# facebookresearch/SlowFast

Measured on AMD Instinct MI355X. Metric: clips/sec (fwd+bwd), SlowFast-8x8-R50 32x224^2 synthetic clips, per-GPU batch 32, higher is better.
Workload: dtype fp16; 1 GPU; SLOWFAST_8x8_R50: forward + cross_entropy loss + backward + sgd step, inputs resident in HBM, per-GPU batch 32; global_batch=32, parallelism=dp1, launch=hip-graph(fwd+bwd) + eager all-reduce/optimizer, optimizer=FlatOptimizer (fused unscale+norm+clip+update, dynamic loss scale on device)

## Files before the change

include/sfamd.h:

```cpp
#ifndef SFAMD_H
#define SFAMD_H
#include <stddef.h>
#include <stdint.h>
#ifdef __cplusplus
extern "C" {
#endif

#define SF_ABI_VERSION 32
typedef void* sf_stream_t;

typedef struct sf_conv_desc {
    int32_t N, Ci, Ti, Hi, Wi;
    int32_t Co, To, Ho, Wo;
    int32_t kT, kH, kW;
    int32_t sT, sH, sW;
    int32_t pT, pH, pW;
    int32_t dT, dH, dW;
    int32_t Cw;
    int32_t ldx, ldy;
    int32_t Cow;
} sf_conv_desc;

int sf_abi_version(void);
const char* sf_backend(void);
#define SF_ACT_FP16 0
#define SF_ACT_BF16_ID 1
int sf_act_dtype(void);
const char* sf_last_error(void);
const char* sf_build_id(void);

int sf_conv_weight_ld(const sf_conv_desc* d, int32_t* ldf, int32_t* ldd);
int sf_prep_weights(const sf_conv_desc* d, const float* w, void* wf, void* wd, sf_stream_t stream);
typedef struct sf_prep_item {
    const float* w;
    void* wf;
    void* wd;
    int32_t Co, Cow, Cw, Cp, taps, ldf, ldd;
    int32_t pad;
} sf_prep_item;
int sf_prep_item_fill(const sf_conv_desc* d, const float* w, void* wf, void* wd, sf_prep_item* item);
int64_t sf_prep_item_blocks(const sf_prep_item* item);
// ... 286 lines not shown
```

slowfast_amd/csrc/sf_api.hip:

```cpp
#include "../../include/sfamd.h"
#include "sf_bn.h"
#include "sf_common.h"
#include "sf_igemm.h"
#include "sf_igemm2.h"
#include "sf_wgrad2.h"
#include "sf_cbwd.h"
#include "sf_pool.h"
#include "sf_dwconv.h"
#include "sf_dwsweep.h"
#include "sf_dwtemporal.h"
#include "sf_tokens.h"
#include "sf_x3d.h"
#include "sf_stem.h"
#include "sf_attn.h"
#include "sf_roi.h"
#include "sf_optim.h"
#include "sf_mixup.h"
#include "sf_erase.h"
#include "sf_pack.h"
#include "sf_sample.h"
#include "sf_color.h"
#include "sf_randaug.h"
#include "sf_hog.h"
#include "sf_pixel.h"
// ... 837 lines not shown
    r.lanes = lanes;
    const int per_block = SF_THREADS / lanes;
    hipLaunchKernelGGL(sf_wgrad_reduce_kernel, dim3(cdiv(total, per_block)), dim3(SF_THREADS), 0, s, r);
    return check_launch("wgrad_reduce");
}

struct CbwdPlan {
    bool ok;
    int cip, cop, R;
    size_t ws_bytes;
};
#define SF_CBWD_MAX_WGS 1024
template <int CIP, int COP>
static void cbwd_fill(CbwdPlan& w) {
    using K = CbwdCfg<CIP, COP>;
    w.R = K::R;
    w.ws_bytes = (size_t)SF_CBWD_MAX_WGS * COP * CIP * 4;
}
#define SF_CBWD_FOR_SHAPE(cip, cop, ...)                                                         \
    do {                                                                                         \
        if ((cip) == 16 && (cop) == 32) { constexpr int CIP_ = 16, COP_ = 32; __VA_ARGS__; }            \
        else if ((cip) == 16 && (cop) == 64) { constexpr int CIP_ = 16, COP_ = 64; __VA_ARGS__; }       \
        else if ((cip) == 16 && (cop) == 128) { constexpr int CIP_ = 16, COP_ = 128; __VA_ARGS__; }     \
        else if ((cip) == 16 && (cop) == 256) { constexpr int CIP_ = 16, COP_ = 256; __VA_ARGS__; }     \
        else if ((cip) == 32 && (cop) == 32) { constexpr int CIP_ = 32, COP_ = 32; __VA_ARGS__; }       \
        else if ((cip) == 32 && (cop) == 64) { constexpr int CIP_ = 32, COP_ = 64; __VA_ARGS__; }       \
        else if ((cip) == 32 && (cop) == 128) { constexpr int CIP_ = 32, COP_ = 128; __VA_ARGS__; }     \
        else if ((cip) == 32 && (cop) == 256) { constexpr int CIP_ = 32, COP_ = 256; __VA_ARGS__; }     \
        else if ((cip) == 64 && (cop) == 32) { constexpr int CIP_ = 64, COP_ = 32; __VA_ARGS__; }       \
        else if ((cip) == 64 && (cop) == 64) { constexpr int CIP_ = 64, COP_ = 64; __VA_ARGS__; }       \
        else if ((cip) == 64 && (cop) == 128) { constexpr int CIP_ = 64, COP_ = 128; __VA_ARGS__; }     \
        else { constexpr int CIP_ = 64, COP_ = 256; __VA_ARGS__; }                                      \
    } while (0)
static CbwdPlan plan_cbwd(const sf_conv_desc* d, bool in_affine, bool mask_bits) {
    CbwdPlan w;
    memset(&w, 0, sizeof(w));
    if (test_hook("SF_CBWD", 1) == 0) return w;
    if (d->kT != 1 || d->kH != 1 || d->kW != 1 || d->sT != 1 || d->sH != 1 || d->sW != 1 || d->pT || d->pH || d->pW) return w;
    if (d->To != d->Ti || d->Ho != d->Hi || d->Wo != d->Wi) return w;
    if (d->Ci % 8 || d->Ci > 64 || d->Co % 32 || d->Co > 256) return w;
    if (in_affine || !mask_bits) return w;
    w.cip = d->Ci <= 16 ? 16 : d->Ci <= 32 ? 32 : 64;
    w.cop = d->Co <= 32 ? 32 : d->Co <= 64 ? 64 : d->Co <= 128 ? 128 : 256;
    SF_CBWD_FOR_SHAPE(w.cip, w.cop, (cbwd_fill<CIP_, COP_>(w)));
    w.ok = true;
    return w;
}

extern "C" int sf_conv_c_bwd_plan(const sf_conv_desc* d, int in_affine, int mask_bits, int32_t* tile_rows,
                                  int64_t* workspace_bytes) {
    if (check_desc(d)) return -1;
    const CbwdPlan w = plan_cbwd(d, in_affine != 0, mask_bits != 0);
    if (tile_rows) *tile_rows = w.ok ? 128 : 0;
    if (workspace_bytes) *workspace_bytes = w.ok ? (int64_t)w.ws_bytes : 0;
    return w.ok ? 1 : 0;
}

extern "C" int sf_conv_c_bwd(const sf_conv_desc* d, const void* dz, int32_t lddz, const void* mask_bits, const void* yc,
                             int32_t ldyc, const float* coef, const void* act, const void* wd, const float* bn_scale,
                             const float* bn_shift, const void* bn_y, int32_t bn_ldy, float* bn_part, int32_t bn_part_rows,
                             int32_t* bn_rows, void* d_in, int32_t ld_in, float* dw, float out_scale, int zero_first,
                             void* workspace, int64_t workspace_bytes, sf_stream_t stream) {
    if (check_desc(d)) return -1;
    REQUIRE(dz && mask_bits && yc && coef && act && wd && d_in && dw && workspace, "sf_conv_c_bwd: null pointer");
    const CbwdPlan w = plan_cbwd(d, false, true);
    REQUIRE(w.ok, "sf_conv_c_bwd: this geometry keeps sf_bn_bwd_apply + sf_conv_wgrad + sf_conv_dgrad_bn (sf_conv_c_bwd_plan == 0)");
    REQUIRE(lddz >= d->Co && lddz % 8 == 0 && ldyc >= d->Co && ldyc % 8 == 0 && ld_in >= d->Ci && ld_in % 8 == 0,
            "sf_conv_c_bwd: bad row pitch");
    REQUIRE((((uintptr_t)dz | (uintptr_t)yc | (uintptr_t)act | (uintptr_t)wd | (uintptr_t)d_in | (uintptr_t)workspace) & 15) == 0,
            "sf_conv_c_bwd: operands must be 16-byte aligned");
    REQUIRE(workspace_bytes >= (int64_t)w.ws_bytes, "sf_conv_c_bwd: workspace too small (%lld < %lld bytes)",
            (long long)workspace_bytes, (long long)w.ws_bytes);
    const int64_t M = (int64_t)d->N * d->Ti * d->Hi * d->Wi;
    const int ntiles = cdiv(M, 128);
    const bool fuse = bn_part != nullptr;
    if (fuse) {
        REQUIRE(bn_scale && bn_shift && bn_y && bn_rows, "sf_conv_c_bwd: the fused reduction needs bn_scale, bn_shift, bn_y and bn_rows");
        REQUIRE(bn_ldy >= d->Ci && bn_ldy % 8 == 0 && ((uintptr_t)bn_y & 15) == 0, "sf_conv_c_bwd: bad bn_y pitch / alignment");
        REQUIRE(bn_part_rows >= ntiles, "sf_conv_c_bwd: the partial table needs ceil(positions / tile_rows) rows of [2][Ci] floats");
    }
    int32_t ldf, ldd;
    sf_conv_weight_ld(d, &ldf, &ldd);
    CbwdParams p;
    memset(&p, 0, sizeof(p));
    p.M = (int)M; p.Ci = d->Ci; p.Co = d->Co;
    p.dz = (const f16*)dz; p.lddz = lddz; p.bits = (const uint8_t*)mask_bits; p.yc = (const f16*)yc; p.ldyc = ldyc;
    p.coef = coef; p.act = (const f16*)act; p.ldact = d->ldx; p.wd = (const f16*)wd; p.ldw = ldd;
    if (fuse) { p.bnb_y = (const f16*)bn_y; p.bnb_ld = bn_ldy; p.bnb_scale = bn_scale; p.bnb_shift = bn_shift; p.bnb_part = bn_part; }
    p.dx = (f16*)d_in; p.lddx = ld_in; p.ws = (float*)workspace; p.tiles128 = ntiles;
    int wgs;
    const Wgrad2Plan w2 = plan_wgrad2(d);
    const int forced = test_hook("SF_CBWD_WGS", 0);
    if (forced > 0) {
        wgs = forced < SF_CBWD_MAX_WGS ? forced : SF_CBWD_MAX_WGS;
        p.rps = roundup(cdiv(M, wgs), 32);
        wgs = cdiv(M, p.rps);
    } else if (w2.ok && w2.thin && w2.splits <= SF_CBWD_MAX_WGS) {
        wgs = w2.splits; p.rps = 0;
    } else {
        const WgradPlan w1 = plan_wgrad(d);
        wgs = w1.splits; p.rps = w1.chunks_per_split * 32;
        REQUIRE(wgs <= SF_CBWD_MAX_WGS, "sf_conv_c_bwd: %d splits", wgs);
    }
    hipStream_t s = (hipStream_t)stream;
    SF_CBWD_FOR_SHAPE(w.cip, w.cop, hipLaunchKernelGGL((sf_cbwd_kernel<CIP_, COP_>), dim3(wgs), dim3(SF_THREADS), 0, s, p));
    if (check_launch("conv_c_bwd")) return -1;
    if (bn_rows) *bn_rows = fuse ? ntiles : 0;
    WgradReduceParams r;
    memset(&r, 0, sizeof(r));
    r.ws = (const float*)workspace; r.splits = wgs; r.Co = d->Cow ? d->Cow : d->Co; r.Co_pad = w.cop; r.Kpad = w.cip;
    r.Ktot = d->Ci; r.fdC = make_fastdiv(d->Ci); r.dw = dw; r.Cw = d->Cw; r.taps = 1; r.slice4 = 0;
    r.out_scale = out_scale; r.accumulate = zero_first ? 0 : 1;
    const int64_t total = (int64_t)r.Co * r.Kpad / 4;
    int lanes = 1;
    while (lanes < 32 && lanes * 4 <= r.splits) lanes *= 2;
    r.lanes = lanes;
    hipLaunchKernelGGL(sf_wgrad_reduce_kernel, dim3(cdiv(total, SF_THREADS / lanes)), dim3(SF_THREADS), 0, s, r);
    return check_launch("conv_c_bwd_reduce");
}

static RowTile make_rowtile(int64_t M, int C, int max_blocks, dim3& grid) {
    RowTile rt;
    rt.M = (int)M; rt.C = C;
    const int G = C / 8;
    const int TG = G < SF_THREADS ? G : SF_THREADS;
    const int rpi = SF_THREADS / TG;
    int passes = cdiv(M, (int64_t)rpi * max_blocks);
    if (passes < 1) passes = 1;
    rt.rows_per_block = rpi * passes;
    grid = dim3(cdiv(M, rt.rows_per_block), cdiv(G, SF_THREADS));
    return rt;
}
static int check_rows(const char* who, int64_t M, int C) {
    REQUIRE(M > 0 && M < (1ll << 31), "%s: bad row count", who);
    REQUIRE(C > 0 && C % 8 == 0, "%s: C must be a positive multiple of 8 (got %d)", who, C);
    return 0;
}

// ... 2264 lines not shown
```

slowfast_amd/csrc/sf_cbwd.h:

```cpp
#pragma once
#include "sf_bn.h"
#include "sf_common.h"
#include "sf_igemm.h"

struct CbwdParams {
    int M, Ci, Co;
    const f16* dz; int lddz;
    const uint8_t* bits;
    const f16* yc; int ldyc;
    const float* coef;
    const f16* act; int ldact;
    const f16* wd; int ldw;
    const f16* bnb_y; int bnb_ld;
    const float* bnb_scale; const float* bnb_shift;
    float* bnb_part;
    f16* dx; int lddx;
    float* ws;
    int rps;
    int tiles128;
};

template <int CIP, int COP>
struct CbwdCfg {
    static constexpr int R = COP >= 128 ? 64 : 128;
    static constexpr int NSUB = 128 / R;
    static constexpr int NJ = CIP / 16, KS = COP / 32, TI = R / 64;
    static constexpr int WAVES_M = COP == 32 ? 4 : 1, WAVES_C = 4 / WAVES_M;
    static constexpr int TC = COP / 16 / WAVES_C;
    static constexpr int KSM = R / WAVES_M / 32;
    static constexpr int LDY = COP + 8;
    static constexpr int CGO = COP / 8, RPP = SF_THREADS / CGO, NCH = R / RPP;
    static constexpr int ACH = CIP / 8, NACT = R * ACH / 64;
    static constexpr int NEPI = (R * ACH + SF_THREADS - 1) / SF_THREADS;
    static constexpr int DY_ELEMS = R * LDY, ACT_ELEMS = R * CIP, WD_ELEMS = CIP * LDY;
    static constexpr int RED_ELEMS = 4 * ACH * 24 * 2;
    static constexpr int UNION_ELEMS = DY_ELEMS > ACT_ELEMS + RED_ELEMS ? DY_ELEMS : ACT_ELEMS + RED_ELEMS;
    static constexpr int LDS_ELEMS = UNION_ELEMS + ACT_ELEMS + WD_ELEMS + 3 * COP * 2 + 2 * CIP * 2;
    static_assert(WAVES_M == 1 || LDS_ELEMS * 2 >= 4 * (COP / 16) * NJ * 256 * 4, "the cross-wave sum reuses the tile buffers");
    static constexpr int LDS_BYTES = LDS_ELEMS * 2;
    static constexpr int HELD = 4 * NJ * (TI + TC) + 9 * NCH + 4 * NEPI;
    static constexpr int OCC = HELD <= 72 ? 3 : 2;
    static_assert(R % 64 == 0 && R % RPP == 0 && NACT >= 1 && (R * ACH) % 64 == 0, "tile shape");
    static_assert(SF_THREADS % ACH == 0 && 64 % ACH == 0, "a thread keeps one d_in column group");
};

template <int CIP, int COP>
__global__ __launch_bounds__(SF_THREADS, (CbwdCfg<CIP, COP>::OCC)) void sf_cbwd_kernel(CbwdParams p) {
    using K = CbwdCfg<CIP, COP>;
    constexpr int R = K::R, LDY = K::LDY, NJ = K::NJ, TI = K::TI, TC = K::TC;
    __shared__ __attribute__((aligned(16))) f16 smem[K::LDS_ELEMS];
    f16* const DyL = smem;
    f16* const StL = smem;
    float* const red = reinterpret_cast<float*>(smem + K::ACT_ELEMS);
    f16* const ActL = smem + K::UNION_ELEMS;
    f16* const WdL = ActL + K::ACT_ELEMS;
    float* const coefL = reinterpret_cast<float*>(WdL + K::WD_ELEMS);
    float* const bnL = coefL + 3 * COP;

    const int tid = threadIdx.x;
    const int lane = tid & 63, wave = __builtin_amdgcn_readfirstlane(tid >> 6);
    const int pl = lane & 15, g4 = lane >> 4;
    const int G = (int)gridDim.x;
    const f16* const zline = reinterpret_cast<const f16*>(sf_zero_line);
    const bool bnb = p.bnb_part != nullptr;

    for (int q = tid; q < CIP * K::CGO; q += SF_THREADS) {
        const int ci = q / K::CGO, cg = q % K::CGO;
        f16x8 v = zero8();
        if (ci < p.Ci && cg * 8 < p.Co) v = ld16(p.wd + (int64_t)ci * p.ldw + cg * 8);
        st16(WdL + ci * LDY + cg * 8, v);
    }
    for (int q = tid; q < 3 * COP; q += SF_THREADS) {
        const int k = q / COP, c = q % COP;
        coefL[q] = c < p.Co ? p.coef[k * p.Co + c] : 0.f;
    }
    for (int q = tid; q < 2 * CIP; q += SF_THREADS) {
        const int k = q / CIP, c = q % CIP;
        bnL[q] = (bnb && c < p.Ci) ? (k ? p.bnb_shift[c] : p.bnb_scale[c]) : (k ? 0.f : 1.f);
    }

    const int scg = tid % K::CGO, srow = tid / K::CGO;
    const bool scol_ok = scg * 8 < p.Co;
    const int scgc = scol_ok ? scg : 0;
    const int ecg = tid % K::ACH;
    const bool ecol_ok = ecg * 8 < p.Ci;
    const int ecgc = ecol_ok ? ecg : 0;

    int r0 = 0, r1 = p.M, T0 = (int)blockIdx.x, Tstep = G, nwalk = 0;
    if (p.rps > 0) {
        r0 = (int)blockIdx.x * p.rps;
        r1 = r0 + p.rps < p.M ? r0 + p.rps : p.M;
        T0 = r0 >> 7;
        Tstep = 1;
        if (r1 > r0) nwalk = (((r1 + 127) >> 7) - T0) * K::NSUB;
    } else if (T0 < p.tiles128) nwalk = ((p.tiles128 - 1 - T0) / G + 1) * K::NSUB;
    auto tile_m0 = [&](int q) { return (T0 + (q / K::NSUB) * Tstep) * 128 + (q % K::NSUB) * R; };

    f16x8 dzr[K::NCH], ycr[K::NCH], ybr[K::NEPI];
    uint32_t mbr[K::NCH];
    auto load_regs = [&](int m0) {
#pragma unroll
        for (int u = 0; u < K::NCH; ++u) {
            int m = m0 + srow + u * K::RPP;
            if (m > p.M - 1) m = p.M - 1;
            dzr[u] = ld16(p.dz + (int64_t)m * p.lddz + scgc * 8);
            ycr[u] = ld16(p.yc + (int64_t)m * p.ldyc + scgc * 8);
            mbr[u] = p.bits[(int64_t)m * (p.Co >> 3) + scgc];
        }
    };
    auto load_yb = [&](int m0) {
#pragma unroll
        for (int e = 0; e < K::NEPI; ++e) {
            int m = m0 + (tid + e * SF_THREADS) / K::ACH;
            if (m > p.M - 1) m = p.M - 1;
            ybr[e] = ld16(p.bnb_y + (int64_t)m * p.bnb_ld + ecgc * 8);
        }
    };
    auto issue_act = [&](int m0) {
#pragma unroll
        for (int j = 0; j < (K::NACT + 3) / 4; ++j) {
            const int q = wave + 4 * j;
            if (q < K::NACT) {
                const int c = q * 64 + lane;
                const int m = m0 + c / K::ACH, cc = c % K::ACH;
                const f16* g = (m >= r0 && m < r1 && cc * 8 < p.Ci) ? p.act + (int64_t)m * p.ldact + cc * 8 : zline;
                SF_GLOBAL_LOAD_LDS16_ASM(g, ActL + q * 512);
            }
        }
    };


    f32x4 wacc[TC][NJ];
#pragma unroll
    for (int i = 0; i < TC; ++i)
#pragma unroll
        for (int j = 0; j < NJ; ++j) wacc[i][j] = (f32x4){0.f, 0.f, 0.f, 0.f};
    const int wc = wave % K::WAVES_C, wm = wave / K::WAVES_C;
    const int cobase = wc * TC * 16, mbase = wm * (R / K::WAVES_M);
    const int rowbase = wave * (R / 4);

    float bsg[8], bsgy[8];
#pragma unroll
    for (int e = 0; e < 8; ++e) { bsg[e] = 0.f; bsgy[e] = 0.f; }
    const int nq = nwalk;
    if (nq > 0) { load_regs(tile_m0(0)); issue_act(tile_m0(0)); }
    for (int q = 0; q < nq; ++q) {
        const int m0 = tile_m0(q);
        const int T = T0 + (q / K::NSUB) * Tstep;
        const bool owner = T * 128 >= r0 && T * 128 < r1;
        const bool more = q + 1 < nq;
        SF_WAIT_VMEM();
        __syncthreads();
        {
            float k1[8], k2[8], k3[8];
#pragma unroll
            for (int e = 0; e < 8; ++e) { k1[e] = coefL[scg * 8 + e]; k2[e] = coefL[COP + scg * 8 + e]; k3[e] = coefL[2 * COP + scg * 8 + e]; }
#pragma unroll
            for (int u = 0; u < K::NCH; ++u) {
                const int row = srow + u * K::RPP;
                const uint32_t b = mbr[u];
                const f16x8 yv = ycr[u];
                float g[8];
#pragma unroll
                for (int e = 0; e < 8; ++e) g[e] = (float)dzr[u][e];
#pragma unroll
                for (int e = 0; e < 8; ++e) g[e] = ((b >> e) & 1u) ? g[e] : 0.f;
                f16x8 o;
#pragma unroll
                for (int e = 0; e < 8; ++e) o[e] = (f16)(k1[e] * g[e] + k2[e] + k3[e] * (float)yv[e]);
                if (!(scol_ok && m0 + row < p.M)) o = zero8();
                st16(DyL + row * LDY + scg * 8, o);
            }
        }
        __syncthreads();
        if (more) load_regs(tile_m0(q + 1));
#pragma unroll
        for (int ks = 0; ks < K::KSM; ++ks) {
            f16x8 af[TC], bf[NJ];
#pragma unroll
            for (int h = 0; h < 2; ++h) {
                const int m = mbase + ks * 32 + 8 * g4 + 4 * h + (pl >> 2);
#pragma unroll
                for (int i = 0; i < TC; ++i) {
                    const f16x4 v = as_f16x4(SF_LDS_TR16(DyL + m * LDY + cobase + i * 16 + 4 * (pl & 3)));
                    af[i][4 * h + 0] = v[0]; af[i][4 * h + 1] = v[1]; af[i][4 * h + 2] = v[2]; af[i][4 * h + 3] = v[3];
                }
#pragma unroll
                for (int j = 0; j < NJ; ++j) {
                    const f16x4 v = as_f16x4(SF_LDS_TR16(ActL + m * CIP + j * 16 + 4 * (pl & 3)));
                    bf[j][4 * h + 0] = v[0]; bf[j][4 * h + 1] = v[1]; bf[j][4 * h + 2] = v[2]; bf[j][4 * h + 3] = v[3];
                }
            }
#pragma unroll
            for (int i = 0; i < TC; ++i)
#pragma unroll
                for (int j = 0; j < NJ; ++j) wacc[i][j] = SF_MFMA16(af[i], bf[j], wacc[i][j]);
        }
        SF_BARRIER_KEEP_VMEM();
        if (more) issue_act(tile_m0(q + 1));
        if (!owner) continue;
        if (bnb) load_yb(m0);
        f32x4 dacc[TI][NJ];
#pragma unroll
        for (int i = 0; i < TI; ++i)
#pragma unroll
            for (int j = 0; j < NJ; ++j) dacc[i][j] = (f32x4){0.f, 0.f, 0.f, 0.f};
#pragma unroll
        for (int ks = 0; ks < K::KS; ++ks) {
            f16x8 bf[NJ];
#pragma unroll
            for (int j = 0; j < NJ; ++j) bf[j] = ld16(WdL + (j * 16 + pl) * LDY + ks * 32 + 8 * g4);
#pragma unroll
            for (int i = 0; i < TI; ++i) {
                const f16x8 af = ld16(DyL + (rowbase + i * 16 + pl) * LDY + ks * 32 + 8 * g4);
#pragma unroll
                for (int j = 0; j < NJ; ++j) dacc[i][j] = SF_MFMA16(af, bf[j], dacc[i][j]);
            }
        }
        SF_BARRIER_KEEP_VMEM();
#pragma unroll
        for (int i = 0; i < TI; ++i)
#pragma unroll
            for (int j = 0; j < NJ; ++j)
#pragma unroll
                for (int r = 0; r < 4; ++r) StL[(rowbase + i * 16 + 4 * g4 + r) * CIP + j * 16 + pl] = (f16)dacc[i][j][r];
        SF_BARRIER_KEEP_VMEM();
        float bsc[8], bsh[8];
#pragma unroll
        for (int e = 0; e < 8; ++e) { bsc[e] = bnL[ecg * 8 + e]; bsh[e] = bnL[CIP + ecg * 8 + e]; }
#pragma unroll
        for (int e = 0; e < K::NEPI; ++e) {
            const int idx = tid + e * SF_THREADS;
            const int row = idx / K::ACH, m = m0 + row;
            if (idx < R * K::ACH && m < p.M && ecol_ok) {
                const f16x8 v = ld16(StL + row * CIP + ecg * 8);
                st16(p.dx + (int64_t)m * p.lddx + ecg * 8, v);
                if (bnb) bnb_accumulate(v, ybr[e], bsc, bsh, bsg, bsgy, false, 0u);
            }
        }
        if (bnb && q % K::NSUB == K::NSUB - 1) {
            bnb_reduce_store<4, K::ACH>(bsg, bsgy, red, p.bnb_part + (int64_t)T * 2 * p.Ci, 0, p.Ci);
#pragma unroll
            for (int e = 0; e < 8; ++e) { bsg[e] = 0.f; bsgy[e] = 0.f; }
        }
    }

    float* slab = p.ws + (int64_t)blockIdx.x * (COP * CIP);
    if constexpr (K::WAVES_M == 4) {
        __syncthreads();
        float* rd = reinterpret_cast<float*>(smem);
#pragma unroll
        for (int i = 0; i < TC; ++i)
#pragma unroll
            for (int j = 0; j < NJ; ++j)
#pragma unroll
                for (int r = 0; r < 4; ++r) rd[(((wave * TC + i) * NJ + j) * 4 + r) * 64 + lane] = wacc[i][j][r];
        __syncthreads();
        constexpr int TE = TC * NJ * 256;
// ... 16 lines not shown
```

slowfast_amd/engine.py:

```python
import functools
import os

import torch

from . import lib as _sflib

from . import ops

_f16 = _sflib.act_dtype()
_listeners = []
FORCE_WEIGHT_PREP = False
PARAM_EPOCH = 0
PACK_RECORD = None
PACK_PLAN = os.environ.get("SF_PACK_PLAN", "1") != "0"
BN_FUSE_REDUCE = os.environ.get("SF_BN_FUSE_REDUCE", "1") != "0"
CAT_IN_PLACE = os.environ.get("SF_CAT_IN_PLACE", "1") != "0"
SEGMENTS = None


class _Segments:
    def __init__(self):
        self.cuts = []

    def cut(self, tensors):
# ... 336 lines not shown
        bn = self.bn
        if bn is None:
            y, _ = ops.conv_fwd(x, wf, geom, in_affine=in_affine, bias=self.conv.bias, stats=False)
            return y, None
        use_batch_stats = training or bn.running_mean is None
        y, part = ops.conv_fwd(x, wf, geom, in_affine=in_affine, bias=self.conv.bias, stats=use_batch_stats)
        return y, bn_statistics(bn, part, geom.out_rows, geom.Co, training)

    def backward(self, x, in_affine, dy, need_dx, resid=None, resid_bits=None, bn_fuse=None):
        geom = self.geom(x.shape)
        w = self.conv.weight
        if w.requires_grad:
            dw, zero_first = _grad_dest(w)
            ops.conv_wgrad(x, dy, geom, dw, in_affine=in_affine, out_scale=1.0, zero_first=zero_first)
        if not need_dx:
            return None
        _, wd = self.weights(geom)
        if bn_fuse is not None:
            if isinstance(bn_fuse, dict):
                return ops.conv_dgrad(dy, wd, geom, resid=resid, resid_bits=resid_bits, bn=bn_fuse)
            y, st = bn_fuse
            return ops.conv_dgrad(dy, wd, geom, resid=resid, bn=(y, st.scale, st.shift))
        return ops.conv_dgrad(dy, wd, geom, resid=resid, resid_bits=resid_bits)

    def _bn_grad_dest(self):
        bn = self.bn
        if bn.weight.requires_grad:
            dgamma, zg = _grad_dest(bn.weight)
            dbeta, zb = _grad_dest(bn.bias)
            assert zg == zb
            return dgamma, dbeta, not zg
        return torch.empty_like(bn.weight), torch.empty_like(bn.bias), False

    def fused_c_geom(self, x):
        if self.bn is None or _sync_of(self.bn) is not None or not self.conv.weight.requires_grad:
            return None
        geom = self.geom(x.shape)
        return geom if ops.conv_c_bwd_plan(geom) is not None else None

    def fused_c_backward(self, geom, x, dz, y, st, bits, part=None, bn_fuse=None):
        bn = self.bn
        dgamma, dbeta, accumulate = self._bn_grad_dest()
        coef = ops.bn_bwd_coef(dz, y, bn.weight, st.mean, st.rstd, dgamma, dbeta, zmask=bits, inv_loss_scale=1.0,
                               accumulate=accumulate, part=part)
        dw, zero_first = _grad_dest(self.conv.weight)
        _, wd = self.weights(geom)
        fuse = None
        if bn_fuse is not None:
            y0, st0 = bn_fuse
            fuse = (y0, st0.scale, st0.shift)
        return ops.conv_c_bwd(dz, bits, y, coef, x, wd, geom, dw, bn=fuse, out_scale=1.0, zero_first=zero_first)

    def bn_backward(self, dz, y, st, zmask=None, relu_self=False, want_g=False, part=None):
        bn = self.bn
        dgamma, dbeta, accumulate = self._bn_grad_dest()
        return ops.bn_bwd(dz, y, bn.weight, st.mean, st.rstd, dgamma, dbeta, zmask=zmask,
                          relu_affine=(st.scale, st.shift) if relu_self else None, inv_loss_scale=1.0,
                          accumulate=accumulate, want_g=want_g, sync=_sync_of(bn), part=part)

    def params(self):
        p = [self.conv.weight]
        if self.conv.bias is not None:
            p.append(self.conv.bias)
        if self.bn is not None:
            p += [self.bn.weight, self.bn.bias]
        return p

    def _fold_source(self, w):
        return w

    def fold(self):
        w = self.conv.weight.detach().float()
        b = self.conv.bias.detach().float() if self.conv.bias is not None else None
        bn = self.bn
        if bn is not None:
            assert bn.running_mean is not None, "BatchNorm without running statistics cannot be folded"
            scale = torch.rsqrt(bn.running_var.detach().float() + bn.eps)
            if bn.weight is not None:
                scale = scale * bn.weight.detach().float()
            shift = -bn.running_mean.detach().float() * scale
            if bn.bias is not None:
                shift = shift + bn.bias.detach().float()
            w = w * scale.view(-1, 1, 1, 1, 1)
            b = shift if b is None else b * scale + shift
# ... 135 lines not shown
            ops.bn_act(x_s, out=cat[:, :Cs])
        ops.bn_act(yf, st.scale, st.shift, relu=True, out=cat[:, Cs:])
        if CAPTURE is not None:
            CAPTURE.append({"kind": "fuse", "mod": mod, "raw": [yf], "bn": [(st.scale, st.shift)]})
        ctx.mod, ctx.yf, ctx.st, ctx.Cs = mod, yf, st, Cs
        ctx.save_for_backward(x_f)
        return cat, x_f.view_as(x_f)

    @staticmethod
    @delivers_grads
    def backward(ctx, dcat, dxf):
        unit = ctx.mod._unit
        (x_f,) = ctx.saved_tensors
        dcat = as_cl(dcat)
        dyf = unit.bn_backward(dcat[:, ctx.Cs:], ctx.yf, ctx.st, relu_self=True)
        need_dx = ctx.needs_input_grad[1]
        dx_f = unit.backward(x_f, None, dyf, need_dx=need_dx, resid=as_cl(dxf) if dxf is not None else None)
        _notify(unit.params())
        ctx.yf = None
        dx_s = dcat[:, :ctx.Cs] if ctx.needs_input_grad[0] else None
        return (dx_s, dx_f, None) + param_grads(ctx, 3)


class ResBlockFn(torch.autograd.Function):

    @staticmethod
    def forward(ctx, x, mod, *params):
        record_params(ctx, params)
        ctx.prev_bn = getattr(x, "_sf_block_bn", None) if BN_FUSE_REDUCE else None
        x = as_cl(x)
        units, P = mod.branch2._chain, mod._proj
        tr = mod.training
        raw, bn, act, h = [], [], [], x
        for i, u in enumerate(units):
            h, st = u.forward(h, None, tr)
            raw.append(h)
            bn.append(st)
            if i + 1 < len(units):
                h = ops.bn_act(h, st.scale, st.shift, relu=True)
                act.append(h)
        yc, sc = raw[-1], bn[-1]
        out_view, cat = None, None
        extra = getattr(mod, "_cat_extra", 0)
        if extra and CAT_IN_PLACE:
            N_, C_, T_, H_, W_ = yc.shape
            cat = ops.cl_empty((N_, C_ + extra, T_, H_, W_), x.device)
            out_view = cat[:, :C_]
        if P is not None:
            y1, s1 = P.forward(x, None, tr)
            out, bits = ops.bn_act(yc, sc.scale, sc.shift, relu=True, resid=y1, rscale=s1.scale, rshift=s1.shift,
                                   want_mask=True, out=out_view)
        else:
            y1, s1 = None, None
            out, bits = ops.bn_act(yc, sc.scale, sc.shift, relu=True, resid=x, want_mask=True, out=out_view)
        if cat is not None:
            out._sf_cat = cat
        if CAPTURE is not None:
            CAPTURE.append({"kind": "resblock", "mod": mod, "raw": list(raw), "bn": [(b.scale, b.shift) for b in bn], "out": out})
        ctx.mod = mod
        ctx.raw = (raw, y1, act, bits)
        ctx.bn = (bn, s1)
        ctx.save_for_backward(x)
        if BN_FUSE_REDUCE and tr:
            out._sf_block_bn = {"bits": bits, "y0": yc, "sync": _sync_of(units[-1].bn) is not None}
        return out

    @staticmethod
    @delivers_grads
    def backward(ctx, dout):
        mod = ctx.mod
        units, P = mod.branch2._chain, mod._proj
        (x,) = ctx.saved_tensors
        raw, y1, act, bits = ctx.raw
        bn, s1 = ctx.bn
        last = len(units) - 1
        part_c = tagged_bn_part(dout, raw[last])
        dout = as_cl(dout)
        need_dx = ctx.needs_input_grad[0]
        cgeom = units[last].fused_c_geom(act[last - 1]) if last > 0 else None
        if cgeom is None:
            dy = units[last].bn_backward(dout, raw[last], bn[last], zmask=bits, part=part_c)
        if P is not None:
            dy1 = P.bn_backward(dout, y1, s1, zmask=bits)
        for i in range(last, 0, -1):
            part = None
            if i == last and cgeom is not None:
                inner = (raw[i - 1], bn[i - 1]) if BN_FUSE_REDUCE and _sync_of(units[i - 1].bn) is None else None
                d_in, part = units[i].fused_c_backward(cgeom, act[i - 1], dout, raw[i], bn[i], bits, part=part_c, bn_fuse=inner)
            elif BN_FUSE_REDUCE and _sync_of(units[i - 1].bn) is None:
                d_in, part = units[i].backward(act[i - 1], None, dy, need_dx=True, bn_fuse=(raw[i - 1], bn[i - 1]))
            else:
                d_in = units[i].backward(act[i - 1], None, dy, need_dx=True)
            dy = units[i - 1].bn_backward(d_in, raw[i - 1], bn[i - 1], relu_self=True, part=part)
        prev = ctx.prev_bn if need_dx else None
        if prev is not None and prev["sync"]:
            prev = None
        if P is not None:
            dx1 = P.backward(x, None, dy1, need_dx=need_dx)
            dx = units[0].backward(x, None, dy, need_dx=need_dx, resid=dx1, bn_fuse=prev)
        else:
            dx = units[0].backward(x, None, dy, need_dx=need_dx, resid=dout, resid_bits=bits, bn_fuse=prev)
        if prev is not None:
            dx, pc = dx
            if pc is not None:
                tag_bn_part(dx, prev["y0"], pc)
        _notify(mod._param_list)
        ctx.raw = ctx.bn = ctx.prev_bn = None
        return (dx, None) + param_grads(ctx, 2)


CUT_BACKWARD = False
_cut_bn_tags = {}


def retag_cut_grad(g):
    tag = _cut_bn_tags.pop(g.data_ptr(), None)
    if tag is not None and getattr(g, "_sf_bn_part", None) is None and tag[2] == g.data_ptr() and tag[3] == g._version:
        g._sf_bn_part = tag


def tag_bn_part(dx, y0, part):
    dx._sf_bn_part = (y0.data_ptr(), part, dx.data_ptr(), dx._version)
    if CUT_BACKWARD:
        _cut_bn_tags[dx.data_ptr()] = dx._sf_bn_part


def tagged_bn_part(dout, y0):
    tag = getattr(dout, "_sf_bn_part", None)
    if tag is None or tag[0] != y0.data_ptr() or tag[2] != dout.data_ptr() or tag[3] != dout._version:
        return None
    return tag[1]


class ConvBNActFn(torch.autograd.Function):

    @staticmethod
    def forward(ctx, x, unit, relu, training, *params):
        record_params(ctx, params)
        x = as_cl(x)
        y, st = unit.forward(x, None, training)
# ... 18 lines not shown
```

slowfast_amd/lib.py:

```python
import ctypes
import os
from ctypes import POINTER, Structure, c_char_p, c_float, c_int, c_int32, c_int64, c_void_p

_HERE = os.path.dirname(os.path.abspath(__file__))
ABI_VERSION = 32
ACT_MODE = os.environ.get("SF_ACT_DTYPE", "fp16").lower()
if ACT_MODE not in ("fp16", "bf16"):
    raise ValueError(f"SF_ACT_DTYPE={ACT_MODE!r}: expected fp16 or bf16")
DEFAULT_LIBRARY = os.path.join(_HERE, "libsfamd.so" if ACT_MODE == "fp16" else "libsfamd_bf16.so")


def act_dtype():
    import torch
    return torch.float16 if ACT_MODE == "fp16" else torch.bfloat16


def act_eps():
    return 2.0 ** -11 if ACT_MODE == "fp16" else 2.0 ** -8


class ConvDesc(Structure):

    _fields_ = [(n, c_int32) for n in (
        "N", "Ci", "Ti", "Hi", "Wi", "Co", "To", "Ho", "Wo", "kT", "kH", "kW", "sT", "sH", "sW",
        "pT", "pH", "pW", "dT", "dH", "dW", "Cw", "ldx", "ldy", "Cow")]


class PrepItem(Structure):

    _fields_ = [("w", c_void_p), ("wf", c_void_p), ("wd", c_void_p)] + [(n, c_int32) for n in (
        "Co", "Cow", "Cw", "Cp", "taps", "ldf", "ldd", "pad")]


class DwDesc(Structure):

    _fields_ = [(n, c_int32) for n in (
        "N", "C", "Cw", "cls", "Ti", "Hi", "Wi", "To", "Ho", "Wo", "kT", "kH", "kW", "sT", "sH", "sW",
        "pT", "pH", "pW", "ldx", "ldy", "Cwreal")]
# ... 237 lines not shown
```

slowfast_amd/ops.py:

```python
from ctypes import byref, c_int32, c_int64

import torch

from . import lib as _sflib

from .lib import ConvDesc, SfError, get_lib

_f16 = _sflib.act_dtype()


def _triple(v):
    return tuple(v) if isinstance(v, (tuple, list)) else (v, v, v)


def _stream(t):
    if t.is_cuda:
        return torch.cuda.current_stream(t.device).cuda_stream
    if get_lib().backend != "hostsim":
        raise SfError("slowfast_amd kernels need CUDA/HIP tensors (got a CPU tensor and the gfx950 library)")
    return None


def _ptr(t):
    return None if t is None else t.data_ptr()
# ... 326 lines not shown
        import torch.distributed as dist
        group, gsize = sync
        tot = part.sum(0, keepdim=True)
        loc = tot.clone()
        lib.call("sf_bn_bwd_finalize", loc.data_ptr(), 1, C, gamma.numel(), float(M), gamma.data_ptr(), mean.data_ptr(),
                 rstd.data_ptr(), float(inv_loss_scale), dgamma.data_ptr(), dbeta.data_ptr(), int(accumulate),
                 coef.data_ptr(), s)
        dist.all_reduce(tot, group=group)
        scratch = torch.empty((2, gamma.numel()), dtype=torch.float32, device=y.device)
        lib.call("sf_bn_bwd_finalize", tot.data_ptr(), 1, C, gamma.numel(), float(M) * gsize, gamma.data_ptr(),
                 mean.data_ptr(), rstd.data_ptr(), float(inv_loss_scale), scratch[0].data_ptr(), scratch[1].data_ptr(), 0,
                 coef.data_ptr(), s)
    if coef_only:
        return coef
    dy = cl_empty(y.shape, y.device) if out is None else out
    if sample_add is not None:
        assert fused_part is not None and zmask is None and relu_affine is None and not want_g
        assert sample_add.dtype == torch.float32 and sample_add.is_contiguous() and tuple(sample_add.shape) == (N, C)
        lib.call("sf_bn_bwd_apply_sample", M, C, dz.data_ptr(), lddz, y.data_ptr(), ldy, coef.data_ptr(), sample_add.data_ptr(),
                 M // N, dy.data_ptr(), cl_ld(dy), s, work=dict(bytes=2.0 * y.numel() * 3))
        return dy
    g = cl_empty(y.shape, y.device) if want_g else None
    lib.call("sf_bn_bwd_apply", M, C, dz.data_ptr(), lddz, _ptr(zmask), ldm, y.data_ptr(), ldy, _ptr(sc), _ptr(sh),
             relu_self, coef.data_ptr(), dy.data_ptr(), cl_ld(dy), _ptr(g), cl_ld(g) if g is not None else 0, s,
             work=dict(bytes=2.0 * y.numel() * (3 + mcost + int(want_g))))
    return (dy, g) if want_g else dy


def bn_bwd_coef(dz, y, gamma, mean, rstd, dgamma, dbeta, zmask=None, inv_loss_scale=1.0, accumulate=False, part=None):
    return bn_bwd(dz, y, gamma, mean, rstd, dgamma, dbeta, zmask=zmask, inv_loss_scale=inv_loss_scale, accumulate=accumulate,
                  part=part, coef_only=True)


def conv_c_bwd_plan(geom, in_affine=False, mask_bits=True):
    tile_rows, ws = c_int32(0), c_int64(0)
    ok = get_lib().call("sf_conv_c_bwd_plan", byref(geom.desc(geom.Ci, geom.Co)), int(bool(in_affine)), int(bool(mask_bits)),
                        byref(tile_rows), byref(ws))
    return (tile_rows.value, ws.value) if ok == 1 else None


def conv_c_bwd(dz, bits, yc, coef, act, wd, geom, dw, bn=None, out_scale=1.0, zero_first=True, out=None):
    plan = conv_c_bwd_plan(geom)
    assert plan is not None, "conv_c_bwd: the planner rejects this geometry"
    tile_rows, ws_bytes = plan
    assert tuple(act.shape) == geom.in_shape and tuple(dz.shape) == geom.out_shape and tuple(yc.shape) == geom.out_shape
    assert dw.dtype == torch.float32 and dw.is_contiguous() and dw.numel() == geom.Cow * geom.Cw * geom.taps
    M = rows(yc)
    assert bits.dtype == torch.uint8 and bits.is_contiguous() and bits.numel() == M * (geom.Co // 8)
    assert coef.dtype == torch.float32 and coef.is_contiguous() and tuple(coef.shape) == (3, geom.Co)
    d_in = cl_empty(geom.in_shape, dz.device) if out is None else out
    assert tuple(d_in.shape) == geom.in_shape
    part, cap, nrows = None, 0, c_int32(0)
    y0 = sc = sh = None
    if bn is not None:
        y0, sc, sh = bn
        assert tuple(y0.shape) == geom.in_shape
        cap = (M + tile_rows - 1) // tile_rows
        part = torch.empty((cap, 2, geom.Ci), dtype=torch.float32, device=dz.device)
    ws = _workspace(dz.device, ws_bytes)
    W = 2.0 * M * geom.Co
    get_lib().call("sf_conv_c_bwd", byref(geom.desc(cl_ld(act), geom.Co)), dz.data_ptr(), cl_ld(dz), bits.data_ptr(), yc.data_ptr(),
                   cl_ld(yc), coef.data_ptr(), act.data_ptr(), wd.data_ptr(), _ptr(sc), _ptr(sh), _ptr(y0),
                   cl_ld(y0) if y0 is not None else 0, _ptr(part), cap, byref(nrows), d_in.data_ptr(), cl_ld(d_in), dw.data_ptr(),
                   float(out_scale), int(zero_first), ws.data_ptr(), ws.numel(), _stream(dz),
                   work=dict(flops=4.0 * M * geom.Co * geom.Cw,
                             bytes=W * (2 + 1 / 16) + 2.0 * M * geom.Ci * (2 + int(bn is not None))))
    return d_in, (part[:nrows.value] if part is not None and nrows.value > 0 else None)


def _pool_args(y, kernel, stride, padding):
    N, C, T, H, W = y.shape
    (kH, kW), (sH, sW), (pH, pW) = kernel, stride, padding
    return (N, T, H, W, C, kH, kW, sH, sW, pH, pW), ((H + 2 * pH - kH) // sH + 1, (W + 2 * pW - kW) // sW + 1)


def pool_fwd(y, kernel, stride, padding, affine=None, want_argmax=True):
    args, (Ho, Wo) = _pool_args(y, kernel, stride, padding)
    N, C, T, H, W = y.shape
    out = cl_empty((N, C, T, Ho, Wo), y.device)
    arg = torch.empty((N, T, Ho, Wo, C), dtype=torch.uint8, device=y.device) if want_argmax else None
    sc, sh, relu = _affine(affine)
    get_lib().call("sf_pool_fwd", *args, y.data_ptr(), cl_ld(y), _ptr(sc), _ptr(sh), relu, out.data_ptr(),
                   cl_ld(out), _ptr(arg), 0, _stream(y), work=dict(bytes=2.0 * (y.numel() + out.numel())))
    return out, arg


def pool_bwd(in_shape, pooled, argmax, dout, kernel, stride, padding, relu=True):
    N, C, T, H, W = in_shape
    (kH, kW), (sH, sW), (pH, pW) = kernel, stride, padding
    assert tuple(dout.shape) == tuple(pooled.shape)
    g = cl_empty(in_shape, dout.device)
    get_lib().call("sf_pool_bwd", N, T, H, W, C, kH, kW, sH, sW, pH, pW, pooled.data_ptr(), cl_ld(pooled),
                   argmax.data_ptr(), int(bool(relu)), dout.data_ptr(), cl_ld(dout), g.data_ptr(), cl_ld(g), 0,
                   _stream(dout), work=dict(bytes=2.0 * (g.numel() + 2.5 * dout.numel())))
    return g
```

Measured before the change: 904.9 clips/s.

## Fold input BN+ReLU into last-unit conv forward and fused backward kernel

In each residual block the last 1x1 conv no longer consumes a materialised BN+ReLU activation. The forward conv takes the affine+relu as an input transform. The fused conv/BN backward kernel gains an AFF variant that recomputes the activation from the raw pre-BN tensor and BN scale/shift into LDS, prefetching the next tile's raw rows. This removes one activation write in forward and one stored tensor, trading it for extra per-element affine work in backward and a different prefetch schedule.

```diff
diff --git a/include/sfamd.h b/include/sfamd.h
--- a/include/sfamd.h
+++ b/include/sfamd.h
@@ -6,7 +6,7 @@
 extern "C" {
 #endif
 
-#define SF_ABI_VERSION 32
+#define SF_ABI_VERSION 33
 typedef void* sf_stream_t;
 
 typedef struct sf_conv_desc {
diff --git a/slowfast_amd/csrc/sf_api.hip b/slowfast_amd/csrc/sf_api.hip
--- a/slowfast_amd/csrc/sf_api.hip
+++ b/slowfast_amd/csrc/sf_api.hip
@@ -893,25 +893,31 @@
         else if ((cip) == 64 && (cop) == 128) { constexpr int CIP_ = 64, COP_ = 128; __VA_ARGS__; }     \
         else { constexpr int CIP_ = 64, COP_ = 256; __VA_ARGS__; }                                      \
     } while (0)
-static CbwdPlan plan_cbwd(const sf_conv_desc* d, bool in_affine, bool mask_bits) {
+static CbwdPlan plan_cbwd_geom(const sf_conv_desc* d) {
     CbwdPlan w;
     memset(&w, 0, sizeof(w));
-    if (test_hook("SF_CBWD", 1) == 0) return w;
     if (d->kT != 1 || d->kH != 1 || d->kW != 1 || d->sT != 1 || d->sH != 1 || d->sW != 1 || d->pT || d->pH || d->pW) return w;
     if (d->To != d->Ti || d->Ho != d->Hi || d->Wo != d->Wi) return w;
     if (d->Ci % 8 || d->Ci > 64 || d->Co % 32 || d->Co > 256) return w;
-    if (in_affine || !mask_bits) return w;
     w.cip = d->Ci <= 16 ? 16 : d->Ci <= 32 ? 32 : 64;
     w.cop = d->Co <= 32 ? 32 : d->Co <= 64 ? 64 : d->Co <= 128 ? 128 : 256;
     SF_CBWD_FOR_SHAPE(w.cip, w.cop, (cbwd_fill<CIP_, COP_>(w)));
     w.ok = true;
     return w;
 }
+static CbwdPlan plan_cbwd(const sf_conv_desc* d, int in_affine, bool mask_bits) {
+    CbwdPlan none;
+    memset(&none, 0, sizeof(none));
+    if (test_hook("SF_CBWD", 1) == 0 || !mask_bits) return none;
+    if (in_affine != 0 && in_affine != 2) return none;
+    if (in_affine == 2 && test_hook("SF_CBWD_AFFINE", 1) == 0) return none;
+    return plan_cbwd_geom(d);
+}
 
 extern "C" int sf_conv_c_bwd_plan(const sf_conv_desc* d, int in_affine, int mask_bits, int32_t* tile_rows,
                                   int64_t* workspace_bytes) {
     if (check_desc(d)) return -1;
-    const CbwdPlan w = plan_cbwd(d, in_affine != 0, mask_bits != 0);
+    const CbwdPlan w = plan_cbwd(d, in_affine, mask_bits != 0);
     if (tile_rows) *tile_rows = w.ok ? 128 : 0;
     if (workspace_bytes) *workspace_bytes = w.ok ? (int64_t)w.ws_bytes : 0;
     return w.ok ? 1 : 0;
@@ -923,8 +929,9 @@
                              int32_t* bn_rows, void* d_in, int32_t ld_in, float* dw, float out_scale, int zero_first,
                              void* workspace, int64_t workspace_bytes, sf_stream_t stream) {
     if (check_desc(d)) return -1;
-    REQUIRE(dz && mask_bits && yc && coef && act && wd && d_in && dw && workspace, "sf_conv_c_bwd: null pointer");
-    const CbwdPlan w = plan_cbwd(d, false, true);
+    REQUIRE(dz && mask_bits && yc && coef && wd && d_in && dw && workspace, "sf_conv_c_bwd: null pointer");
+    const bool aff = act == nullptr;
+    const CbwdPlan w = plan_cbwd_geom(d);
     REQUIRE(w.ok, "sf_conv_c_bwd: this geometry keeps sf_bn_bwd_apply + sf_conv_wgrad + sf_conv_dgrad_bn (sf_conv_c_bwd_plan == 0)");
     REQUIRE(lddz >= d->Co && lddz % 8 == 0 && ldyc >= d->Co && ldyc % 8 == 0 && ld_in >= d->Ci && ld_in % 8 == 0,
             "sf_conv_c_bwd: bad row pitch");
@@ -935,9 +942,10 @@
     const int64_t M = (int64_t)d->N * d->Ti * d->Hi * d->Wi;
     const int ntiles = cdiv(M, 128);
     const bool fuse = bn_part != nullptr;
+    REQUIRE(!aff || (bn_scale && bn_shift && bn_y), "sf_conv_c_bwd: without act, bn_scale, bn_shift and bn_y are what it is formed from");
+    if (fuse || aff) REQUIRE(bn_ldy >= d->Ci && bn_ldy % 8 == 0 && ((uintptr_t)bn_y & 15) == 0, "sf_conv_c_bwd: bad bn_y pitch / alignment");
     if (fuse) {
         REQUIRE(bn_scale && bn_shift && bn_y && bn_rows, "sf_conv_c_bwd: the fused reduction needs bn_scale, bn_shift, bn_y and bn_rows");
-        REQUIRE(bn_ldy >= d->Ci && bn_ldy % 8 == 0 && ((uintptr_t)bn_y & 15) == 0, "sf_conv_c_bwd: bad bn_y pitch / alignment");
         REQUIRE(bn_part_rows >= ntiles, "sf_conv_c_bwd: the partial table needs ceil(positions / tile_rows) rows of [2][Ci] floats");
     }
     int32_t ldf, ldd;
@@ -947,7 +955,7 @@
     p.M = (int)M; p.Ci = d->Ci; p.Co = d->Co;
     p.dz = (const f16*)dz; p.lddz = lddz; p.bits = (const uint8_t*)mask_bits; p.yc = (const f16*)yc; p.ldyc = ldyc;
     p.coef = coef; p.act = (const f16*)act; p.ldact = d->ldx; p.wd = (const f16*)wd; p.ldw = ldd;
-    if (fuse) { p.bnb_y = (const f16*)bn_y; p.bnb_ld = bn_ldy; p.bnb_scale = bn_scale; p.bnb_shift = bn_shift; p.bnb_part = bn_part; }
+    if (fuse || aff) { p.bnb_y = (const f16*)bn_y; p.bnb_ld = bn_ldy; p.bnb_scale = bn_scale; p.bnb_shift = bn_shift; p.bnb_part = bn_part; }
     p.dx = (f16*)d_in; p.lddx = ld_in; p.ws = (float*)workspace; p.tiles128 = ntiles;
     int wgs;
     const Wgrad2Plan w2 = plan_wgrad2(d);
@@ -964,7 +972,8 @@
         REQUIRE(wgs <= SF_CBWD_MAX_WGS, "sf_conv_c_bwd: %d splits", wgs);
     }
     hipStream_t s = (hipStream_t)stream;
-    SF_CBWD_FOR_SHAPE(w.cip, w.cop, hipLaunchKernelGGL((sf_cbwd_kernel<CIP_, COP_>), dim3(wgs), dim3(SF_THREADS), 0, s, p));
+    if (aff) SF_CBWD_FOR_SHAPE(w.cip, w.cop, hipLaunchKernelGGL((sf_cbwd_kernel<CIP_, COP_, true>), dim3(wgs), dim3(SF_THREADS), 0, s, p));
+    else SF_CBWD_FOR_SHAPE(w.cip, w.cop, hipLaunchKernelGGL((sf_cbwd_kernel<CIP_, COP_>), dim3(wgs), dim3(SF_THREADS), 0, s, p));
     if (check_launch("conv_c_bwd")) return -1;
     if (bn_rows) *bn_rows = fuse ? ntiles : 0;
     WgradReduceParams r;
diff --git a/slowfast_amd/csrc/sf_cbwd.h b/slowfast_amd/csrc/sf_cbwd.h
--- a/slowfast_amd/csrc/sf_cbwd.h
+++ b/slowfast_amd/csrc/sf_cbwd.h
@@ -40,11 +40,12 @@
     static constexpr int LDS_BYTES = LDS_ELEMS * 2;
     static constexpr int HELD = 4 * NJ * (TI + TC) + 9 * NCH + 4 * NEPI;
     static constexpr int OCC = HELD <= 72 ? 3 : 2;
+    static constexpr bool YB_LATE = CIP == 64;
     static_assert(R % 64 == 0 && R % RPP == 0 && NACT >= 1 && (R * ACH) % 64 == 0, "tile shape");
     static_assert(SF_THREADS % ACH == 0 && 64 % ACH == 0, "a thread keeps one d_in column group");
 };
 
-template <int CIP, int COP>
+template <int CIP, int COP, bool AFF = false>
 __global__ __launch_bounds__(SF_THREADS, (CbwdCfg<CIP, COP>::OCC)) void sf_cbwd_kernel(CbwdParams p) {
     using K = CbwdCfg<CIP, COP>;
     constexpr int R = K::R, LDY = K::LDY, NJ = K::NJ, TI = K::TI, TC = K::TC;
@@ -76,7 +77,7 @@
     }
     for (int q = tid; q < 2 * CIP; q += SF_THREADS) {
         const int k = q / CIP, c = q % CIP;
-        bnL[q] = (bnb && c < p.Ci) ? (k ? p.bnb_shift[c] : p.bnb_scale[c]) : (k ? 0.f : 1.f);
+        bnL[q] = ((bnb || AFF) && c < p.Ci) ? (k ? p.bnb_shift[c] : p.bnb_scale[c]) : (k ? 0.f : 1.f);
     }
 
     const int scg = tid % K::CGO, srow = tid / K::CGO;
@@ -96,7 +97,7 @@
     } else if (T0 < p.tiles128) nwalk = ((p.tiles128 - 1 - T0) / G + 1) * K::NSUB;
     auto tile_m0 = [&](int q) { return (T0 + (q / K::NSUB) * Tstep) * 128 + (q % K::NSUB) * R; };
 
-    f16x8 dzr[K::NCH], ycr[K::NCH], ybr[K::NEPI];
+    f16x8 dzr[K::NCH], ycr[K::NCH], ybr[K::NEPI], ybn[AFF ? K::NEPI : 1];
     uint32_t mbr[K::NCH];
     auto load_regs = [&](int m0) {
 #pragma unroll
@@ -108,12 +109,12 @@
             mbr[u] = p.bits[(int64_t)m * (p.Co >> 3) + scgc];
         }
     };
-    auto load_yb = [&](int m0) {
+    auto load_yb = [&](int m0, f16x8* dst) {
 #pragma unroll
         for (int e = 0; e < K::NEPI; ++e) {
             int m = m0 + (tid + e * SF_THREADS) / K::ACH;
             if (m > p.M - 1) m = p.M - 1;
-            ybr[e] = ld16(p.bnb_y + (int64_t)m * p.bnb_ld + ecgc * 8);
+            dst[e] = ld16(p.bnb_y + (int64_t)m * p.bnb_ld + ecgc * 8);
         }
     };
     auto issue_act = [&](int m0) {
@@ -143,7 +144,11 @@
 #pragma unroll
     for (int e = 0; e < 8; ++e) { bsg[e] = 0.f; bsgy[e] = 0.f; }
     const int nq = nwalk;
-    if (nq > 0) { load_regs(tile_m0(0)); issue_act(tile_m0(0)); }
+    if (nq > 0) {
+        load_regs(tile_m0(0));
+        if constexpr (AFF) load_yb(tile_m0(0), ybn);
+        else issue_act(tile_m0(0));
+    }
     for (int q = 0; q < nq; ++q) {
         const int m0 = tile_m0(q);
         const int T = T0 + (q / K::NSUB) * Tstep;
@@ -151,6 +156,18 @@
         const bool more = q + 1 < nq;
         SF_WAIT_VMEM();
         __syncthreads();
+        if constexpr (AFF) {
+#pragma unroll
+            for (int e = 0; e < K::NEPI; ++e) {
+                ybr[e] = ybn[e];
+                const int idx = tid + e * SF_THREADS;
+                const int row = idx / K::ACH, m = m0 + row;
+                f16x8 a = bn_act8(ybn[e], bnL + ecg * 8, bnL + CIP + ecg * 8, 0.f);
+                if (!(ecol_ok && m >= r0 && m < r1)) a = zero8();
+                if (idx < R * K::ACH) st16(ActL + row * CIP + ecg * 8, a);
+            }
+            __builtin_amdgcn_sched_barrier(0);
+        }
         {
             float k1[8], k2[8], k3[8];
 #pragma unroll
@@ -196,10 +213,15 @@
 #pragma unroll
                 for (int j = 0; j < NJ; ++j) wacc[i][j] = SF_MFMA16(af[i], bf[j], wacc[i][j]);
         }
-        SF_BARRIER_KEEP_VMEM();
-        if (more) issue_act(tile_m0(q + 1));
+        if constexpr (AFF) {
+            if (more && !(K::YB_LATE && owner)) load_yb(tile_m0(q + 1), ybn);
+        } else {
+            SF_BARRIER_KEEP_VMEM();
+            if (more) issue_act(tile_m0(q + 1));
+        }
         if (!owner) continue;
-        if (bnb) load_yb(m0);
+        if constexpr (!AFF)
+            if (bnb) load_yb(m0, ybr);
         f32x4 dacc[TI][NJ];
 #pragma unroll
         for (int i = 0; i < TI; ++i)
@@ -224,6 +246,8 @@
             for (int j = 0; j < NJ; ++j)
 #pragma unroll
                 for (int r = 0; r < 4; ++r) StL[(rowbase + i * 16 + 4 * g4 + r) * CIP + j * 16 + pl] = (f16)dacc[i][j][r];
+        if constexpr (AFF && K::YB_LATE)
+            if (more) load_yb(tile_m0(q + 1), ybn);
         SF_BARRIER_KEEP_VMEM();
         float bsc[8], bsh[8];
 #pragma unroll
diff --git a/slowfast_amd/engine.py b/slowfast_amd/engine.py
--- a/slowfast_amd/engine.py
+++ b/slowfast_amd/engine.py
@@ -392,13 +392,15 @@
             return dgamma, dbeta, not zg
         return torch.empty_like(bn.weight), torch.empty_like(bn.bias), False
 
-    def fused_c_geom(self, x):
+    def fused_c_plan(self, x, in_affine=False):
         if self.bn is None or _sync_of(self.bn) is not None or not self.conv.weight.requires_grad:
             return None
         geom = self.geom(x.shape)
-        return geom if ops.conv_c_bwd_plan(geom) is not None else None
-
-    def fused_c_backward(self, geom, x, dz, y, st, bits, part=None, bn_fuse=None):
+        plan = ops.conv_c_bwd_plan(geom, in_affine=in_affine, in_relu=in_affine)
+        return (geom, plan) if plan is not None else None
+
+    def fused_c_backward(self, cplan, x, dz, y, st, bits, part=None, bn_fuse=None, x_affine=None):
+        geom, plan = cplan
         bn = self.bn
         dgamma, dbeta, accumulate = self._bn_grad_dest()
         coef = ops.bn_bwd_coef(dz, y, bn.weight, st.mean, st.rstd, dgamma, dbeta, zmask=bits, inv_loss_scale=1.0,
@@ -406,10 +408,11 @@
         dw, zero_first = _grad_dest(self.conv.weight)
         _, wd = self.weights(geom)
         fuse = None
-        if bn_fuse is not None:
-            y0, st0 = bn_fuse
+        if bn_fuse is not None or x is None:
+            y0, st0 = bn_fuse if bn_fuse is not None else x_affine
             fuse = (y0, st0.scale, st0.shift)
-        return ops.conv_c_bwd(dz, bits, y, coef, x, wd, geom, dw, bn=fuse, out_scale=1.0, zero_first=zero_first)
+        return ops.conv_c_bwd(dz, bits, y, coef, x, wd, geom, dw, bn=fuse, out_scale=1.0, zero_first=zero_first,
+                              want_part=bn_fuse is not None, plan=plan)
 
     def bn_backward(self, dz, y, st, zmask=None, relu_self=False, want_g=False, part=None):
         bn = self.bn
@@ -611,11 +614,22 @@
         units, P = mod.branch2._chain, mod._proj
         tr = mod.training
         raw, bn, act, h = [], [], [], x
+        last = len(units) - 1
+        cplan, affine = None, None
         for i, u in enumerate(units):
-            h, st = u.forward(h, None, tr)
+            if i == last and last > 0:
+                cplan = u.fused_c_plan(raw[i - 1], in_affine=True) if tr else None
+                if cplan is not None:
+                    affine = (bn[i - 1].scale, bn[i - 1].shift, True)
+                    h = raw[i - 1]
+                else:
+                    h = ops.bn_act(raw[i - 1], bn[i - 1].scale, bn[i - 1].shift, relu=True)
+                    cplan = u.fused_c_plan(h)
+                act.append(None if affine is not None else h)
+            h, st = u.forward(h, affine if i == last else None, tr)
             raw.append(h)
             bn.append(st)
-            if i + 1 < len(units):
+            if i + 1 < last:
                 h = ops.bn_act(h, st.scale, st.shift, relu=True)
                 act.append(h)
         yc, sc = raw[-1], bn[-1]
@@ -637,6 +651,7 @@
         if CAPTURE is not None:
             CAPTURE.append({"kind": "resblock", "mod": mod, "raw": list(raw), "bn": [(b.scale, b.shift) for b in bn], "out": out})
         ctx.mod = mod
+        ctx.cplan = cplan
         ctx.raw = (raw, y1, act, bits)
         ctx.bn = (bn, s1)
         ctx.save_for_backward(x)
@@ -656,16 +671,17 @@
         part_c = tagged_bn_part(dout, raw[last])
         dout = as_cl(dout)
         need_dx = ctx.needs_input_grad[0]
-        cgeom = units[last].fused_c_geom(act[last - 1]) if last > 0 else None
-        if cgeom is None:
+        cplan = ctx.cplan
+        if cplan is None:
             dy = units[last].bn_backward(dout, raw[last], bn[last], zmask=bits, part=part_c)
         if P is not None:
             dy1 = P.bn_backward(dout, y1, s1, zmask=bits)
         for i in range(last, 0, -1):
             part = None
-            if i == last and cgeom is not None:
+            if i == last and cplan is not None:
                 inner = (raw[i - 1], bn[i - 1]) if BN_FUSE_REDUCE and _sync_of(units[i - 1].bn) is None else None
-                d_in, part = units[i].fused_c_backward(cgeom, act[i - 1], dout, raw[i], bn[i], bits, part=part_c, bn_fuse=inner)
+                d_in, part = units[i].fused_c_backward(cplan, act[i - 1], dout, raw[i], bn[i], bits, part=part_c, bn_fuse=inner,
+                                                       x_affine=(raw[i - 1], bn[i - 1]))
             elif BN_FUSE_REDUCE and _sync_of(units[i - 1].bn) is None:
                 d_in, part = units[i].backward(act[i - 1], None, dy, need_dx=True, bn_fuse=(raw[i - 1], bn[i - 1]))
             else:
@@ -684,7 +700,7 @@
             if pc is not None:
                 tag_bn_part(dx, prev["y0"], pc)
         _notify(mod._param_list)
-        ctx.raw = ctx.bn = ctx.prev_bn = None
+        ctx.raw = ctx.bn = ctx.prev_bn = ctx.cplan = None
         return (dx, None) + param_grads(ctx, 2)
 
 
diff --git a/slowfast_amd/lib.py b/slowfast_amd/lib.py
--- a/slowfast_amd/lib.py
+++ b/slowfast_amd/lib.py
@@ -3,7 +3,7 @@
 from ctypes import POINTER, Structure, c_char_p, c_float, c_int, c_int32, c_int64, c_void_p
 
 _HERE = os.path.dirname(os.path.abspath(__file__))
-ABI_VERSION = 32
+ABI_VERSION = 33
 ACT_MODE = os.environ.get("SF_ACT_DTYPE", "fp16").lower()
 if ACT_MODE not in ("fp16", "bf16"):
     raise ValueError(f"SF_ACT_DTYPE={ACT_MODE!r}: expected fp16 or bf16")
diff --git a/slowfast_amd/ops.py b/slowfast_amd/ops.py
--- a/slowfast_amd/ops.py
+++ b/slowfast_amd/ops.py
@@ -382,18 +382,20 @@
                   part=part, coef_only=True)
 
 
-def conv_c_bwd_plan(geom, in_affine=False, mask_bits=True):
+def conv_c_bwd_plan(geom, in_affine=False, mask_bits=True, in_relu=False):
     tile_rows, ws = c_int32(0), c_int64(0)
-    ok = get_lib().call("sf_conv_c_bwd_plan", byref(geom.desc(geom.Ci, geom.Co)), int(bool(in_affine)), int(bool(mask_bits)),
+    ok = get_lib().call("sf_conv_c_bwd_plan", byref(geom.desc(geom.Ci, geom.Co)), (2 if in_relu else 1) if in_affine else 0, int(bool(mask_bits)),
                         byref(tile_rows), byref(ws))
     return (tile_rows.value, ws.value) if ok == 1 else None
 
 
-def conv_c_bwd(dz, bits, yc, coef, act, wd, geom, dw, bn=None, out_scale=1.0, zero_first=True, out=None):
-    plan = conv_c_bwd_plan(geom)
+def conv_c_bwd(dz, bits, yc, coef, act, wd, geom, dw, bn=None, out_scale=1.0, zero_first=True, out=None, want_part=True, plan=None):
+    assert act is not None or bn is not None, "conv_c_bwd: without act, bn = (y, scale, shift) is what it is formed from"
+    if plan is None:
+        plan = conv_c_bwd_plan(geom, in_affine=act is None, in_relu=act is None)
     assert plan is not None, "conv_c_bwd: the planner rejects this geometry"
     tile_rows, ws_bytes = plan
-    assert tuple(act.shape) == geom.in_shape and tuple(dz.shape) == geom.out_shape and tuple(yc.shape) == geom.out_shape
+    assert (act is None or tuple(act.shape) == geom.in_shape) and tuple(dz.shape) == geom.out_shape and tuple(yc.shape) == geom.out_shape
     assert dw.dtype == torch.float32 and dw.is_contiguous() and dw.numel() == geom.Cow * geom.Cw * geom.taps
     M = rows(yc)
     assert bits.dtype == torch.uint8 and bits.is_contiguous() and bits.numel() == M * (geom.Co // 8)
@@ -405,16 +407,17 @@
     if bn is not None:
         y0, sc, sh = bn
         assert tuple(y0.shape) == geom.in_shape
-        cap = (M + tile_rows - 1) // tile_rows
-        part = torch.empty((cap, 2, geom.Ci), dtype=torch.float32, device=dz.device)
+        if want_part or act is not None:
+            cap = (M + tile_rows - 1) // tile_rows
+            part = torch.empty((cap, 2, geom.Ci), dtype=torch.float32, device=dz.device)
     ws = _workspace(dz.device, ws_bytes)
     W = 2.0 * M * geom.Co
-    get_lib().call("sf_conv_c_bwd", byref(geom.desc(cl_ld(act), geom.Co)), dz.data_ptr(), cl_ld(dz), bits.data_ptr(), yc.data_ptr(),
-                   cl_ld(yc), coef.data_ptr(), act.data_ptr(), wd.data_ptr(), _ptr(sc), _ptr(sh), _ptr(y0),
+    get_lib().call("sf_conv_c_bwd", byref(geom.desc(cl_ld(act) if act is not None else geom.Ci, geom.Co)), dz.data_ptr(), cl_ld(dz),
+                   bits.data_ptr(), yc.data_ptr(), cl_ld(yc), coef.data_ptr(), _ptr(act), wd.data_ptr(), _ptr(sc), _ptr(sh), _ptr(y0),
                    cl_ld(y0) if y0 is not None else 0, _ptr(part), cap, byref(nrows), d_in.data_ptr(), cl_ld(d_in), dw.data_ptr(),
                    float(out_scale), int(zero_first), ws.data_ptr(), ws.numel(), _stream(dz),
                    work=dict(flops=4.0 * M * geom.Co * geom.Cw,
-                             bytes=W * (2 + 1 / 16) + 2.0 * M * geom.Ci * (2 + int(bn is not None))))
+                             bytes=W * (2 + 1 / 16) + 2.0 * M * geom.Ci * (1 + int(act is not None) + int(bn is not None))))
     return d_in, (part[:nrows.value] if part is not None and nrows.value > 0 else None)
 
 
```

Result: no change. 910.2 clips/s (median of 6 runs) (+0.6%).
